# JuliaMLTools/GraphNets.jl

Measured on AMD Instinct MI355X. Metric: edges updated/sec, GNBlock fwd, 1M-edge batch, higher is better.
Workload: dtype f32; 1 GPU; C2: one shared Erdos-Renyi graph, 100k nodes / 1M edges, batch_size=1 (BASELINE configs[1]); dims=(10, 5, 0)=>(3, 4, 5), edges_whole_job=1000000, edges_per_gpu=1000000, nodes_per_gpu=100000, graphs_per_gpu=1, parallelism=single GPU

## Files before the change

### graphnets.jl_amd/csrc/gnx_device.h

```cpp
#pragma once
#ifndef GNX_JIT
#include <hip/hip_runtime.h>
#endif

namespace gnx {

struct Tile {
  int n0, n1;
  int e0, e1;
  int g;
  int win0;
  int win1;
  int flags;
};

constexpr int kPdRowsCap = 28;

struct BlockArgs {
  int de, dn, dg;
  int oe, on, og;
  const float *We, *be, *Wn, *bn, *Wg, *bg;
  int act_e, act_n, act_g;
  const float *ef, *nf, *gf;
  float *ef_out, *nf_out, *gf_out;
// ... 5 lines not shown
  const int* edge_off;
  const int* tile_off;
  const Tile* tiles;
  const int* wtile_off;
  const Tile* wtiles;
  int N, E, G, n_tiles, n_wtiles;
  const float* ln_g[3];
  const float* ln_b[3];
  float ln_eps;
  int ln_mode;
  const float* ln_stats[3];
  int ln_inline_e;
  const int* packs;
  int n_packs;
  const float *ffe_w1, *ffe_b1, *ffe_w2, *ffe_b2, *ffe_g2, *ffe_be2;
  int ffe_act1, ffe_act2;
  void* ffe_scratch;
  const float* prev_partials;
  const float* prev_gf;
  float* prev_gf_out;
  int prev_blocks;
};

struct RunSlot {
  const float *ef, *nf, *gf;
  float *ef_out, *nf_out, *gf_out;
  float* partials;
};
constexpr int kRunSlots = 8;
struct RunTable {
  RunSlot slot[kRunSlots];
};
constexpr unsigned kRunTableOffset = (unsigned)((sizeof(BlockArgs) + 7) / 8 * 8);

__device__ __forceinline__ float relu_f(float x) {
  float r;
  asm("v_max_f32 %0, 0, %1" : "=v"(r) : "v"(x));
  return r;
}

__device__ __forceinline__ float act_apply(float x, int act) {
  switch (act) {
    case 1: return relu_f(x);
    case 2: return tanhf(x);
    case 3: return 1.f / (1.f + expf(-x));
    case 4: return 0.5f * x * (1.f + tanhf(0.7978845608028654f * (x + 0.044715f * x * x * x)));
    default: return x;
  }
}

__device__ __forceinline__ float act_grad_from_out(float y, int act) {
  switch (act) {
    case 1: return y > 0.f ? 1.f : 0.f;
    case 2: return 1.f - y * y;
    case 3: return y * (1.f - y);
    default: return 1.f;
  }
}

__device__ __forceinline__ int segment_of(const int* cp, int n, int e) {
  int lo = 0, hi = n;
  while (hi - lo > 1) {
    const int mid = (lo + hi) >> 1;
    if (cp[mid] <= e) lo = mid; else hi = mid;
  }
  return lo;
// ... 10 lines not shown
```

### graphnets.jl_amd/csrc/gnx_forward.hip

```cpp
#include <algorithm>
#include <cstdlib>

#include "gnx_staging.h"
#include "gnx_step_hazard.h"

namespace gnx {

static_assert(GNX_ACT_IDENTITY == 0 && GNX_ACT_RELU == 1 && GNX_ACT_TANH == 2 && GNX_ACT_SIGMOID == 3 && GNX_ACT_GELU == 4,
              "act_apply (gnx_device.h) hard-codes the activation codes");

static int32_t check_block(const gnx_graphs* h, const gnx_block_params* p, int64_t R) {
  if (!h || !p) return fail(GNX_ERR_INVALID_ARG, "NULL handle or params");
  if (R <= 0) return fail(GNX_ERR_INVALID_ARG, "n_replicas must be >= 1");
  if (R > 1 && h->G != 1)
    return fail(GNX_ERR_INVALID_ARG, "n_replicas > 1 needs a single-graph handle (shared adjacency, batch.jl:66)");
  if (R > 65535) return fail(GNX_ERR_TOO_LARGE, "n_replicas exceeds the grid limit (65535)");
  const int d[6] = {p->de, p->dn, p->dg, p->oe, p->on, p->og};
  for (int i = 0; i < 6; ++i)
    if (d[i] < 0) return fail(GNX_ERR_DIMS, "negative feature width");
  if (p->de + p->dn + p->dg == 0) return fail(GNX_ERR_DIMS, "all input widths are 0 (gnblock.jl:48, batch.jl:56)");
  if (p->oe + p->on + p->og == 0) return fail(GNX_ERR_DIMS, "all output widths are 0 (gnblock.jl:49)");
  const gnx_dense* fn[3] = {&p->edgefn, &p->nodefn, &p->graphfn};
  const int out[3] = {p->oe, p->on, p->og};
  const int in[3] = {p->de + 2 * p->dn + p->dg, p->oe + p->dn + p->dg, p->oe + p->on + p->dg};
// ... 329 lines not shown
int32_t gnx_block_forward_chained(const gnx_graphs* h, const gnx_block_params* p, const float* ef, const float* nf, const float* gf, int64_t R, float* ef_out,
                                  float* nf_out, float* gf_out, void* ws, size_t ws_bytes, uint32_t flags, void* stream, const gnx_pending_update* prev,
                                  gnx_pending_update* pending) {
  if (!pending) return fail(GNX_ERR_INVALID_ARG, "pending is NULL");
  DeviceTurn turn((hipStream_t)stream, p && matrix_core_widths(*p));
  if (flags & GNX_FLAG_DEFER_GRAPH_UPDATE) return fail(GNX_ERR_INVALID_ARG, "gnx_block_forward_chained defers the graph update itself");
  return chained_step(BlockCall{h, p, GNX_ELEM_F32, ef, nf, gf, R, ef_out, nf_out, gf_out, ws, ws_bytes, flags, (hipStream_t)stream, GNX_PHASE_ALL}, prev, pending);
}

static StepSpans step_spans(const gnx_graphs* h, const gnx_block_params* p, int64_t R, const gnx_block_step& st, size_t elem, size_t ws_extent) {
  const void* const in[3] = {st.ef, st.nf, st.gf};
  const void* const out[3] = {st.ef_out, st.nf_out, st.gf_out};
  const long long rows[3] = {(long long)h->E, (long long)h->N, (long long)h->G};
  const int in_w[3] = {p->de, p->dn, p->dg}, out_w[3] = {p->oe, p->on, p->og};
  return step_spans_of(in, out, st.workspace, st.workspace_bytes, rows, in_w, out_w, R, elem, ws_extent);
}

static bool steps_overlap_applies(const gnx_graphs* h, const gnx_block_params* p, int64_t R, uint32_t flags, hipStream_t s) {
  if (!h || !p || matrix_core_widths(*p) || (flags & GNX_FLAG_FORCE_GENERIC) || form(GNX_FLAG_NO_FORK) || profile_enabled()) return false;
  if (check_block(h, p, R) != GNX_OK) return false;
  return block_narrow_takes(h, block_probe(h, p), s);
}

constexpr int kStepsRunDefault = 8;
static_assert(kRunMax == kRunSlots, "gnx_step_hazard.h groups what gnx_device.h's table holds");
static int steps_run_max() {
  static const int v = [] {
    const char* e = getenv("GNX_STEPS_RUN_MAX");
    const int n = e && *e ? atoi(e) : kStepsRunDefault;
    return n < 1 ? 1 : (n > kRunMax ? kRunMax : n);
  }();
  return v;
}

static int32_t steps_schedule(const gnx_graphs* h, const gnx_block_params* p, int32_t elem, const gnx_block_step* steps, int64_t n_steps, int64_t R,
                              uint32_t flags, void* stream, bool overlap) {
  const AuxHold hold = overlap ? take_aux(h, true) : AuxHold{};
  const gnx_graphs::AuxSet* aux = hold.set;
  const bool two = aux != nullptr;
  hipStream_t str[2] = {(hipStream_t)stream, aux ? aux->stream : nullptr};
  gnx_pending_update pend[2]{};
  auto flush = [&](int k) -> int32_t {
    if (!pend[k].workspace) return GNX_OK;
    const int32_t rc = graph_update(h, p, elem, pend[k], R, flags, str[k]);
    pend[k] = gnx_pending_update{};
    return rc;
  };
  auto run = [&](const gnx_block_step& st, int k, gnx_pending_update* next) -> int32_t {
    const gnx_pending_update* prev = pend[k].workspace ? &pend[k] : nullptr;
    return chained_step(BlockCall{h, p, elem, st.ef, st.nf, st.gf, R, st.ef_out, st.nf_out, st.gf_out, st.workspace, st.workspace_bytes, flags, str[k], GNX_PHASE_ALL},
                        prev, next);
  };
  const bool bf16 = elem == GNX_ELEM_BF16;
  const bool valid = h && p && check_block(h, p, R) == GNX_OK;
  const size_t elem_bytes = bf16 ? 2 : sizeof(float);
  const size_t ws_extent = !valid ? 0 : bf16 ? typed_ws(h, p, R, true).total : block_ws(h, p, R).total;
  bool can_fuse = valid && R == 1 && !(flags & GNX_FLAG_FORCE_GENERIC) && steps_run_max() > 1 && !profile_enabled();
  auto slot_of = [&](const gnx_block_step& st, RunSlot& sl, BlockArgs* run_args) -> bool {
    Prepared q(BlockCall{h, p, elem, st.ef, st.nf, st.gf, R, st.ef_out, st.nf_out, st.gf_out, st.workspace, st.workspace_bytes, flags, str[0], GNX_PHASE_ALL});
    if (q.rc) return false;
    if (run_args) {
      if (!block_narrow_run_applies(h, q.a, bf16)) return can_fuse = false;
      *run_args = q.a;
    }
    sl = RunSlot{q.a.ef, q.a.nf, q.a.gf, q.a.ef_out, q.a.nf_out, q.a.gf_out, q.a.partials};
    return true;
  };
  if (two) {
    GNX_HIP(hipEventRecord(aux->fork, str[0]));
    GNX_HIP(hipStreamWaitEvent(str[1], aux->fork, 0));
  }
  RunSpans recent[3];
  int32_t rc = GNX_OK;
  int64_t i = 0;
  for (int64_t j = 0; i < n_steps && rc == GNX_OK; ++j) {
    const gnx_block_step& st = steps[i];
    RunSpans cur;
    RunTable tab{};
    BlockArgs run_args{};
    cur.step[0] = valid ? step_spans(h, p, R, st, elem_bytes, ws_extent) : StepSpans{};
    cur.n = 1;
    if (can_fuse && n_steps - i >= 2) {
      RunSpans win = cur;
      while (i + win.n < n_steps) {
        const StepSpans sp = step_spans(h, p, R, steps[i + win.n], elem_bytes, ws_extent);
        if (!run_takes(win, sp, steps_run_max())) break;
        win.step[win.n++] = sp;
      }
      bool ok = window_is_run(win.n, i, n_steps, steps_run_max());
      for (int z = 0; ok && z < win.n; ++z) ok = slot_of(steps[i + z], tab.slot[z], z == 0 ? &run_args : nullptr);
      if (ok) cur = win;
    }
    const int k = two ? (int)(j & 1) : 0, o = k ^ 1;
    StepOrder ord;
    if (two) {
      ord = run_order(cur, recent, j);
    } else {
      ord.flush_own = pend[0].workspace && (pend[0].workspace == st.workspace || (p && p->og > 0 && pend[0].gf_out == st.gf_out) || runs_conflict(cur, recent[0]));
    }
    if ((ord.flush_own || cur.n > 1) && (rc = flush(k))) break;
    if (two && j >= 3) {
      const hipError_t e = hipStreamWaitEvent(str[k], aux->step[(j - 3) & 3], 0);
      if (e != hipSuccess) { rc = hip_fail(e, "gnx_block_forward_steps: ordering a step behind the step three before it"); break; }
    }
    if (ord.after_other) {
      if ((rc = flush(o))) break;
      hipEvent_t ev = o == 1 ? aux->join : aux->fork;
      hipError_t e = hipEventRecord(ev, str[o]);
      if (e == hipSuccess) e = hipStreamWaitEvent(str[k], ev, 0);
      if (e != hipSuccess) { rc = hip_fail(e, "gnx_block_forward_steps: ordering a step behind the other stream"); break; }
    }
    if (cur.n > 1) {
      rc = launch_block_narrow_run(h, run_args, tab, cur.n, str[k], bf16);
    } else {
      gnx_pending_update next{};
      rc = run(st, k, &next);
      if (rc == GNX_OK) pend[k] = next;
    }
    if (rc != GNX_OK) break;
    if (two) {
      if (const hipError_t e = hipEventRecord(aux->step[j & 3], str[k]); e != hipSuccess) { rc = hip_fail(e, "gnx_block_forward_steps: step event"); break; }
    }
    recent[2] = recent[1]; recent[1] = recent[0]; recent[0] = cur;
    i += cur.n;
  }
  const int32_t rf0 = flush(0), rf1 = two ? flush(1) : GNX_OK;
  hipError_t e1 = hipSuccess, e2 = hipSuccess;
  if (two) {
    e1 = hipEventRecord(aux->join, str[1]);
    e2 = hipStreamWaitEvent(str[0], aux->join, 0);
  }
  if (rc) return rc;
  if (rf0) return rf0;
  if (rf1) return rf1;
  GNX_HIP(e1);
  GNX_HIP(e2);
  return GNX_OK;
}

int32_t gnx_block_forward_steps(const gnx_graphs* h, const gnx_block_params* p, const gnx_block_step* steps, int64_t n_steps, int64_t R, uint32_t flags,
                                void* stream) {
  if (n_steps < 0 || (n_steps > 0 && !steps)) return fail(GNX_ERR_INVALID_ARG, "gnx_block_forward_steps: steps is NULL / n_steps is negative");
  if (flags & GNX_FLAG_DEFER_GRAPH_UPDATE) return fail(GNX_ERR_INVALID_ARG, "gnx_block_forward_steps finishes every step's graph update itself");
  DeviceTurn turn((hipStream_t)stream, p && matrix_core_widths(*p));
  FormScope forms(flags);
  return steps_schedule(h, p, GNX_ELEM_F32, steps, n_steps, R, flags, stream, n_steps > 1 && steps_overlap_applies(h, p, R, flags, (hipStream_t)stream));
}

int32_t gnx_block_forward_steps_typed(const gnx_graphs* h, const gnx_block_params* p, int32_t elem, const gnx_block_step* steps, int64_t n_steps, int64_t R,
                                      uint32_t flags, void* stream) {
  if (elem == GNX_ELEM_F32) return gnx_block_forward_steps(h, p, steps, n_steps, R, flags, stream);
  if (elem != GNX_ELEM_BF16) return fail(GNX_ERR_INVALID_ARG, "elem must be GNX_ELEM_F32 or GNX_ELEM_BF16");
  if (flags & GNX_FLAG_DEFER_GRAPH_UPDATE) return fail(GNX_ERR_INVALID_ARG, "gnx_block_forward_steps_typed finishes every step's graph update itself");
  if (n_steps < 0 || (n_steps > 0 && !steps)) return fail(GNX_ERR_INVALID_ARG, "gnx_block_forward_steps_typed: steps is NULL / n_steps is negative");
  for (int64_t i = 0; i < n_steps; ++i) {
    const gnx_block_step& st = steps[i];
    const void* bufs[6] = {st.ef, st.nf, st.gf, st.ef_out, st.nf_out, st.gf_out};
    for (const void* b : bufs)
      if (((uintptr_t)b & 3) != 0) return fail(GNX_ERR_INVALID_ARG, "bf16 feature buffers must be 4-byte aligned (in every step)");
  }
  const hipStream_t s = (hipStream_t)stream;
  DeviceTurn turn(s, p && matrix_core_widths(*p));
  FormScope forms(flags);
  if (!h || !p || check_block(h, p, R) != GNX_OK || !typed_native(h, p, flags, s)) {
    for (int64_t i = 0; i < n_steps; ++i) {
// ... 428 lines not shown
```

### graphnets.jl_amd/csrc/gnx_launchers.h

```cpp
#pragma once
#include "gnx_internal.h"

namespace gnx {

struct EdgeLaunch {
  const Tile* tiles; size_t n_tiles; const float* ef; size_t E;
  struct { const float* stats; const float* g; const float* b; bool inline_stats; float eps; int mode; } ln;
  const float* We; int ldw;
  const float* psrc;
  const float* pdst;
  size_t N; const int* src; const int* dst; int act;
  float* out; float* colsum;
  float* agg_out; size_t n_agg_rows; const int* chunk_row0;
  int64_t R; void* scratch; hipStream_t stream;
};

int32_t launch_block_generic(const BlockArgs& a, int64_t R, int tile_n_cap, hipStream_t s, int phase);
int32_t launch_layernorm2(const float* x, size_t rows, int d, const gnx_layernorm& l1, const gnx_layernorm& l2, float eps, int eps_mode, float* y1, float* y2, hipStream_t s);
int32_t launch_layernorm2_bf16(const void* x, size_t rows, int d, const gnx_layernorm& l1, const gnx_layernorm& l2, float eps, int eps_mode, float* y1, float* y2, hipStream_t s);
int32_t launch_ffn_residual(const float* z, const float* x, size_t rows, int d, const gnx_ffn& ff, float* out, hipStream_t s);
int32_t launch_pad(const gnx_graphs* h, int kind, bool pad, const float* src, int d, int64_t R, float* dst, hipStream_t s);
int32_t launch_calibration(int n, hipStream_t s);
int xent_blocks(int64_t cols);
int32_t launch_xent_backward(const float* logits, const float* targets, int d, int64_t cols, const float* upstream, float* dl, hipStream_t s);
int32_t launch_xent(const float* logits, const float* targets, int d, int64_t cols, float* out, float* ws, hipStream_t s);
int32_t launch_collapse(const gnx_graphs* h, const float* ef, int d, int64_t R, float* out, hipStream_t s);
int32_t launch_collapse_padded(const gnx_graphs* h, const float* ef, int d, int64_t R, float* out, hipStream_t s);
int32_t launch_fn_input(const gnx_graphs* h, int kind, const float* ef, int de, const float* nf, int dn, const float* gf, int dg, int64_t R, float* out, hipStream_t s,
                        bool bf16 = false);

int32_t launch_block_narrow(const gnx_graphs* h, const BlockArgs& a, int64_t R, hipStream_t s, int phase, bool bf16 = false);
void warm_block_narrow(const gnx_graphs* h, const gnx_block_params* p, bool bf16 = false);
bool block_narrow_ready(const gnx_graphs* h, const BlockArgs& a, hipStream_t s);
bool block_narrow_ffe_applies(const gnx_graphs* h, const BlockArgs& a, int act1, int act2);
bool block_narrow_chain_applies(const gnx_graphs* h, const BlockArgs& a, bool bf16 = false);
bool block_narrow_takes(const gnx_graphs* h, const BlockArgs& a, hipStream_t s, bool bf16 = false);
int32_t launch_block_narrow_chained(const gnx_graphs* h, const BlockArgs& a, int64_t R, hipStream_t s, bool bf16);
bool narrow_bf16_aot(const gnx_graphs* h, const BlockArgs& a);
int32_t launch_fused_bf16(const gnx_graphs* h, const BlockArgs& a, int64_t R, hipStream_t s, int phase);
int32_t launch_chained_bf16(const gnx_graphs* h, const BlockArgs& a, int64_t R, hipStream_t s);
bool narrow_bf16_ln_aot(const gnx_graphs* h, const BlockArgs& a);
int32_t launch_ln_bf16(const gnx_graphs* h, const BlockArgs& a, int64_t R, hipStream_t s, int phase);
bool block_narrow_run_applies(const gnx_graphs* h, const BlockArgs& a, bool bf16);
bool narrow_bf16_run(const gnx_graphs* h, const BlockArgs& a);
int32_t launch_block_narrow_run(const gnx_graphs* h, const BlockArgs& a, const RunTable& t, int Z, hipStream_t s, bool bf16);
int32_t launch_run_bf16(const gnx_graphs* h, const BlockArgs& a, const RunTable& t, int Z, hipStream_t s);
bool jit_eligible(const BlockArgs& a, int ept);
int32_t jit_get(const BlockArgs& a, int ept, hipStream_t s, hipFunction_t* block, hipFunction_t* graph, bool bf16 = false);
int32_t jit_get_core_post3(int d0, int d1, int d2, hipStream_t s, hipFunction_t* fn);

bool core_narrow_width(int d);
int32_t launch_ln1_rows(const float* x, size_t rows, int d, const gnx_layernorm& l1, float eps, int eps_mode, float* y, hipStream_t s);
bool core_post3_applies(const size_t rows[3], const int d[3], const gnx_ffn ff[3], bool deferred, hipStream_t s);
int32_t launch_core_post3(const float* const x[3], const size_t rows[3], const int d[3], const gnx_layernorm l2[3], const gnx_ffn ff[3], float eps,
                          int eps_mode, float* const out[3], hipStream_t s, const BlockArgs* blk, int n_rows, bool skip_edges = false,
                          const float* const block_out[3] = nullptr);
int32_t launch_core_post(const float* x, size_t rows, int d, const gnx_layernorm& l2, const gnx_ffn& ff, float eps, int eps_mode, float* out, hipStream_t s,
                         const float* block_out = nullptr);

int32_t launch_block_wide(const gnx_graphs* h, const BlockArgs& a, int64_t R, hipStream_t s, int phase);
size_t wide_workspace_bytes(const gnx_graphs* h, const gnx_block_params* p, int64_t R);
void warm_block_wide(const gnx_graphs* h, const gnx_block_params* p, bool rows_gemm);
bool block_wide_ln_applies(const gnx_graphs* h, const BlockArgs& a);
bool block_wide_edge_x6_applies(const gnx_graphs* h, const BlockArgs& a);
int32_t launch_dense_rows(const gnx_graphs* h, int entity, const float* A, int K, const gnx_dense& d, int OUT, const float* add1,
                          const float* add2, float* out, int64_t R, hipStream_t s, const char* name);
int32_t launch_rows_matmul(const gnx_graphs* h, int entity, const float* A, int K, const float* B, int ldw, int OUT, float* out, int64_t R,
                           hipStream_t s, const char* name, const float* gmul, int gmul_act, float* tile_colsum, int* n_tiles_out, const float* add1);

int32_t launch_ffn_fused(const gnx_graphs* h, int entity, const float* z, int d, const gnx_ffn& ff, const float* add1, const float* add2, float* out,
                         int64_t R, hipStream_t s, const float* ln_stats = nullptr, const gnx_layernorm* ln = nullptr, void* scratch = nullptr, size_t scratch_bytes = 0,
                         bool ln_inline = false, float ln_eps = 0.f, int ln_mode = 0);
bool ffn_fused_applies(const float* z, int d, const gnx_ffn& ff, const float* add1, const float* add2, const float* out);
bool ln_stats_applies(const float* x, int d);
int32_t launch_ln_stats(const float* x, size_t rows, int d, float eps, int eps_mode, float* stats, hipStream_t s);
bool ffn_x6_applies(const float* z, int d, const gnx_ffn& ff, const float* add1, const float* add2, const float* out, size_t scratch_bytes);
int32_t launch_ffn_x6(const float* z, size_t nrows, int d, const gnx_ffn& ff, const float* add1, const float* add2, float* out, int64_t R, hipStream_t s,
                      const float* ln_stats, const gnx_layernorm* ln, void* scratch, bool ln_inline, float ln_eps, int ln_mode);
// ... 80 lines not shown
```

### graphnets.jl_amd/csrc/gnx_narrow.hip

```cpp
#include <cstdlib>

#include "gnx_launchers.h"
#include "gnx_narrow_launch.h"
#include "gnx_wave_kernel.h"

namespace gnx {

#define GNX_NARROW_DIMS(X) \
  X(10, 5, 0, 3, 4)        \
  X(3, 4, 5, 3, 4)         \
  X(10, 5, 3, 3, 4)        \
  X(0, 2, 0, 2, 2)         \
  X(2, 2, 2, 2, 2)         \
  X(4, 3, 2, 3, 4)         \
  X(8, 8, 8, 16, 8)        \
  X(10, 5, 3, 10, 5)       \
  X(10, 5, 0, 10, 5)
static bool narrow_aot_listed(const BlockArgs& a) {
#define GNX_CASE(DE, DN, DG, OE, ON) \
  if (a.de == DE && a.dn == DN && a.dg == DG && a.oe == OE && a.on == ON) return true;
  GNX_NARROW_DIMS(GNX_CASE)
#undef GNX_CASE
  return false;
}
// ... 68 lines not shown
  a.prev_blocks = a.prev_partials ? (h->G == 1 ? 1 : (int)((h->G + 3) / 4)) : 0;
  if (bf16) {
    const int32_t rc = launch_chained_bf16(h, a, R, s);
    return rc == 1 ? fail(GNX_ERR_INVALID_ARG, "internal: chained bf16 launch for a width set without that kernel") : rc;
  }
#define GNX_CASE(DE, DN, DG, OE, ON)                                                                                               \
  if (a.de == DE && a.dn == DN && a.dg == DG && a.oe == OE && a.on == ON) {                                                         \
    if constexpr (OE + ON > 0) {                                                                                                   \
      return h->G == 1 ? launch_wave_g<DE, DN, DG, OE, ON, 2, false, true, false, true>(h, a, R, s, 1)                              \
                       : launch_wave_g<DE, DN, DG, OE, ON, 2, false, false, false, true>(h, a, R, s, 1);                            \
    }                                                                                                                              \
  }
  GNX_NARROW_DIMS(GNX_CASE)
#undef GNX_CASE
  return fail(GNX_ERR_INVALID_ARG, "internal: chained launch for a width set without that kernel");
}

#define GNX_NARROW_RUN_DIMS(X) \
  X(10, 5, 0, 3, 4)            \
  X(3, 4, 5, 3, 4)             \
  X(10, 5, 3, 3, 4)            \
  X(0, 2, 0, 2, 2)             \
  X(2, 2, 2, 2, 2)             \
  X(4, 3, 2, 3, 4)
bool block_narrow_run_applies(const gnx_graphs* h, const BlockArgs& a, bool bf16) {
  if (!block_narrow_chain_applies(h, a, bf16)) return false;
  if (bf16) return narrow_bf16_run(h, a);
#define GNX_CASE(DE, DN, DG, OE, ON) \
  if (a.de == DE && a.dn == DN && a.dg == DG && a.oe == OE && a.on == ON) return true;
  GNX_NARROW_RUN_DIMS(GNX_CASE)
#undef GNX_CASE
  return false;
}
int32_t launch_block_narrow_run(const gnx_graphs* h, const BlockArgs& a, const RunTable& t, int Z, hipStream_t s, bool bf16) {
  if (bf16) {
    const int32_t rc = launch_run_bf16(h, a, t, Z, s);
    return rc == 1 ? fail(GNX_ERR_INVALID_ARG, "internal: bf16 run launch for a width set without that kernel") : rc;
  }
#define GNX_CASE(DE, DN, DG, OE, ON)                                                                                               \
  if (a.de == DE && a.dn == DN && a.dg == DG && a.oe == OE && a.on == ON) {                                                         \
    if constexpr (OE + ON > 0) {                                                                                                   \
      return h->G == 1 ? launch_wave_run<DE, DN, DG, OE, ON, true>(h, a, t, Z, s) : launch_wave_run<DE, DN, DG, OE, ON, false>(h, a, t, Z, s); \
    }                                                                                                                              \
  }
  GNX_NARROW_RUN_DIMS(GNX_CASE)
#undef GNX_CASE
  return fail(GNX_ERR_INVALID_ARG, "internal: run launch for a width set without that kernel");
}

bool block_narrow_ffe_applies(const gnx_graphs* h, const BlockArgs& a, int act1, int act2) {
  return ln_aot(h, a) && a.ln_g[0] && act1 <= GNX_ACT_RELU && act2 <= GNX_ACT_RELU && a.act_e <= GNX_ACT_RELU && h->max_in_degree <= h->wtile_e_cap &&
         !form(GNX_FLAG_NO_FFE);
}

enum NarrowRoute { NR_NONE, NR_AOT, NR_JIT };
static NarrowRoute narrow_route(const gnx_graphs* h, const BlockArgs& a, hipStream_t s, bool bf16 = false) {
  if (a.n_wtiles == 0 || a.E == 0 || wants_ln(a)) return NR_NONE;
  auto jit_ok = [&]() {
    const int ept = jit_ept(h);
    hipFunction_t fb, fg;
    return ept && jit_get(a, ept, s, &fb, &fg, bf16) == GNX_OK;
  };
  static const bool jit_all = getenv("GNX_JIT_ALL") != nullptr;
  if (jit_all && jit_ok()) return NR_JIT;
  if (bf16) {
    if (narrow_bf16_aot(h, a)) return NR_AOT;
  } else if (narrow_aot_listed(a)) {
    return h->wtile_e_cap == 64 || h->wtile_e_cap == 128 || (h->wtile_e_cap == 256 && (a.de + a.dn) * 4 <= 64) ? NR_AOT : NR_NONE;
  }
  return jit_ok() ? NR_JIT : NR_NONE;
}

bool block_narrow_takes(const gnx_graphs* h, const BlockArgs& a, hipStream_t s, bool bf16) { return narrow_route(h, a, s, bf16) != NR_NONE; }

int32_t launch_block_narrow(const gnx_graphs* h, const BlockArgs& a, int64_t R, hipStream_t s, int phase, bool bf16) {
  if (a.n_wtiles == 0 || a.E == 0) return 1;
  if (wants_ln(a)) {
    if (bf16) {
      const int32_t rc = launch_ln_bf16(h, a, R, s, phase);
      return rc == 1 ? fail(GNX_ERR_INVALID_ARG, "internal: LayerNorm-on-load on bf16 rows for a width set without that kernel") : rc;
// ... 25 lines not shown
```

### graphnets.jl_amd/csrc/gnx_narrow_launch.h

```cpp
#pragma once
#include <cstdlib>

#include "gnx_device.h"
#include "gnx_wave_kernel.h"

namespace gnx {

static int partial_rows(const gnx_graphs* h) { return (int)(h->G == 1 ? (h->n_wtiles() + 3) / 4 : h->n_wtiles()); }

static int graph_update_threads(const gnx_graphs* h) {
  return graph_update_threads_for_rows(h->G == 1 ? (h->n_wtiles() + 3) / 4 : h->max_wtiles_per_graph);
}

template <int DE, int DN, int DG, int OE, int ON, int EPT, bool LN, bool ONEG, bool FFE = false, bool CHAIN = false, bool BF16 = false>
static int32_t launch_wave_g(const gnx_graphs* h, const BlockArgs& a, int64_t R, hipStream_t s, int phase) {
  constexpr int C = OE + ON;
  const int n_rows = partial_rows(h);
  const unsigned grid = (unsigned)((a.n_wtiles + 3) / 4) + (CHAIN ? (unsigned)a.prev_blocks : 0u);
  if (phase & 1) {
    ProfScope ps("k_block_wave", s);
#ifdef GNX_WAVE_STAMPS_BUILD
    static unsigned long long* d_dbg = nullptr;
    static size_t dbg_cap = 0;
    const char* dump = getenv("GNX_WAVE_STAMPS_DUMP");
    if (dump) {
      if (dbg_cap < (size_t)a.n_wtiles) { if (d_dbg) (void)hipFree(d_dbg); dbg_cap = (size_t)a.n_wtiles; (void)hipMalloc((void**)&d_dbg, dbg_cap * 64); }
      (void)hipMemsetAsync(d_dbg, 0, (size_t)a.n_wtiles * 64, s);
      (void)hipMemcpyToSymbolAsync(HIP_SYMBOL(g_wave_dbg), &d_dbg, sizeof(d_dbg), 0, hipMemcpyHostToDevice, s);
    }
#endif
    if constexpr (FFE) GNX_LAUNCH((k_block_wave_ffe<DE, DN, DG, OE, ON, EPT, ONEG, BF16>), dim3(grid, (unsigned)R), dim3(kThreads), 0, s, a, n_rows);
    else GNX_LAUNCH((k_block_wave<DE, DN, DG, OE, ON, EPT, LN, ONEG, false, false, CHAIN, BF16>), dim3(grid, (unsigned)R), dim3(kThreads), 0, s, a, n_rows);
    GNX_HIP(hipGetLastError());
#ifdef GNX_WAVE_STAMPS_BUILD
    if (dump) {
      (void)hipStreamSynchronize(s);
      std::vector<unsigned long long> hs((size_t)a.n_wtiles * 8);
      (void)hipMemcpy(hs.data(), d_dbg, hs.size() * 8, hipMemcpyDeviceToHost);
      if (FILE* f = fopen(dump, "wb")) { fwrite(hs.data(), 8, hs.size(), f); fclose(f); }
    }
#endif
  }
  if ((phase & 2) && a.og > 0) {
    if constexpr (C > 0) {
      const int threads = graph_update_threads(h);
      const size_t lds = sizeof(float) * (size_t)graph_update_lds_floats(C, a.dg, a.og, threads);
      ProfScope ps("k_graph_t", s);
      GNX_LAUNCH((k_graph_t<C, ONEG, BF16, BF16 && !LN>), dim3((unsigned)a.G, (unsigned)R), dim3(threads), lds, s, a, n_rows);
      GNX_HIP(hipGetLastError());
    }
  }
  return GNX_OK;
}

template <int DE, int DN, int DG, int OE, int ON, bool ONEG, bool BF16 = false>
static int32_t launch_wave_run(const gnx_graphs* h, const BlockArgs& a, const RunTable& t, int Z, hipStream_t s) {
  constexpr int C = OE + ON;
  if (Z < 1 || Z > kRunSlots) return fail(GNX_ERR_INVALID_ARG, "internal: a run of more steps than the table has slots");
  const int n_rows = partial_rows(h);
  {
    ProfScope ps("k_block_wave", s);
    GNX_LAUNCH((k_block_wave_run<DE, DN, DG, OE, ON, 2, ONEG, BF16>), dim3((unsigned)((a.n_wtiles + 3) / 4), (unsigned)Z), dim3(kThreads), 0, s, a, t, n_rows);
    GNX_HIP(hipGetLastError());
  }
  if (a.og > 0) {
    const int threads = graph_update_threads(h);
    const size_t lds = sizeof(float) * (size_t)graph_update_lds_floats(C, a.dg, a.og, threads);
    ProfScope ps("k_graph_t", s);
    GNX_LAUNCH((k_graph_run<C, ONEG, BF16>), dim3((unsigned)a.G, (unsigned)Z), dim3(threads), lds, s, a, t, n_rows);
    GNX_HIP(hipGetLastError());
  }
  return GNX_OK;
}

template <int DE, int DN, int DG, int OE, int ON, int EPT, bool BF16 = false>
static bool launch_wave_pack(const gnx_graphs* h, const BlockArgs& a, int64_t R, hipStream_t s, int phase, int32_t* rc) {
  constexpr int C = OE + ON;
  if constexpr (EPT != 2 || C == 0) return false;
  else {
    if (h->G <= 1 || h->n_packs <= 0 || !a.packs || phase != 3 || a.og <= 0 || form(GNX_FLAG_NO_PACK)) return false;
    ProfScope ps("k_block_wave", s);
    GNX_LAUNCH((k_block_wave<DE, DN, DG, OE, ON, EPT, false, false, true, false, false, BF16>), dim3((unsigned)h->n_packs, (unsigned)R), dim3(kPackThreads), 0, s, a, 0);
    const hipError_t e = hipGetLastError();
    *rc = e == hipSuccess ? GNX_OK : hip_fail(e, "k_block_wave<PACK>");
    return true;
  }
}

template <int DE, int DN, int DG, int OE, int ON, int EPT, bool LN = false, bool BF16 = false>
static int32_t launch_wave_t(const gnx_graphs* h, const BlockArgs& a, int64_t R, hipStream_t s, int phase) {
  if constexpr (!LN) {
    int32_t rc = GNX_OK;
    if (launch_wave_pack<DE, DN, DG, OE, ON, EPT, BF16>(h, a, R, s, phase, &rc)) return rc;
  }
  return h->G == 1 ? launch_wave_g<DE, DN, DG, OE, ON, EPT, LN, true, false, false, BF16>(h, a, R, s, phase)
                   : launch_wave_g<DE, DN, DG, OE, ON, EPT, LN, false, false, false, BF16>(h, a, R, s, phase);
}

template <int DE, int DN, int DG, int OE, int ON, bool BF16 = false>
static int32_t launch_fused(const gnx_graphs* h, const BlockArgs& a, int64_t R, hipStream_t s, int phase) {
  if (h->wtile_e_cap == 64) return launch_wave_t<DE, DN, DG, OE, ON, 1, false, BF16>(h, a, R, s, phase);
  if (h->wtile_e_cap == 128) return launch_wave_t<DE, DN, DG, OE, ON, 2, false, BF16>(h, a, R, s, phase);
  if (h->wtile_e_cap == 256) {
    if constexpr ((DE + DN) * 4 <= 64) return launch_wave_t<DE, DN, DG, OE, ON, 4, false, BF16>(h, a, R, s, phase);
// ... 6 lines not shown
```

### graphnets.jl_amd/csrc/gnx_step_hazard.h

```cpp
#pragma once
#include <cstddef>
#include <cstdint>

namespace gnx {

struct ByteSpan {
  uintptr_t lo = 0, hi = 0;
};

inline ByteSpan byte_span(const void* p, size_t bytes) {
  ByteSpan s;
  if (p && bytes) { s.lo = reinterpret_cast<uintptr_t>(p); s.hi = s.lo + bytes; }
  return s;
}

inline bool spans_overlap(ByteSpan a, ByteSpan b) { return a.lo < a.hi && b.lo < b.hi && a.lo < b.hi && b.lo < a.hi; }

struct StepSpans {
  ByteSpan rd[3];
  ByteSpan wr[4];
};

inline StepSpans step_spans_of(const void* const in[3], const void* const out[3], const void* ws, size_t ws_bytes, const long long rows[3],
                               const int in_w[3], const int out_w[3], long long R, size_t elem, size_t ws_extent) {
// ... 42 lines not shown
  return false;
}

inline bool runs_conflict(const RunSpans& x, const RunSpans& y) {
  for (int b = 0; b < y.n; ++b)
    if (run_conflicts_step(x, y.step[b])) return true;
  return false;
}

inline bool run_takes(const RunSpans& run, const StepSpans& next, int run_max) {
  return run.n >= 1 && run.n < run_max && run.n < kRunMax && !run_conflicts_step(run, next);
}

inline bool window_is_run(int n, long long first, long long n_steps, int run_max) {
  return n >= 2 && (n == run_max || (first + n == n_steps && n >= kRunTailMin));
}

inline RunSpans group_run(const StepSpans* spans, long long n_steps, long long first, int run_max) {
  RunSpans run;
  if (first >= n_steps) return run;
  run.step[run.n++] = spans[first];
  while (first + run.n < n_steps && run_takes(run, spans[first + run.n], run_max)) { run.step[run.n] = spans[first + run.n]; ++run.n; }
  if (!window_is_run(run.n, first, n_steps, run_max)) run.n = 1;
  return run;
}

inline StepOrder run_order(const RunSpans& cur, const RunSpans* recent, long long j) {
  StepOrder o;
  o.flush_own = j >= 2 && runs_conflict(cur, recent[1]);
  o.after_other = (j >= 1 && runs_conflict(cur, recent[0])) || (j >= 3 && runs_conflict(cur, recent[2]));
  return o;
}

}
```

### graphnets.jl_amd/csrc/gnx_wave_kernel.h

```cpp
#pragma once
#include "gnx_device.h"

namespace gnx {

namespace {

constexpr int kThreads = 256;

struct __attribute__((packed, aligned(4))) F4u { float x, y, z, w; };
struct __attribute__((packed, aligned(4))) F3u { float x, y, z; };
struct __attribute__((packed, aligned(4))) F2u { float x, y; };

typedef const float __attribute__((address_space(4))) * cfloatp;
__device__ __forceinline__ cfloatp as_const(const float* p) { return reinterpret_cast<cfloatp>(reinterpret_cast<size_t>(p)); }

template <int D>
__device__ __forceinline__ void load_row(const float* __restrict__ p, float (&x)[D > 0 ? D : 1]) {
  constexpr int Q = D / 4, R = D % 4;
#pragma unroll
  for (int q = 0; q < Q; ++q) {
    const F4u v = *reinterpret_cast<const F4u*>(p + 4 * q);
    x[4 * q] = v.x; x[4 * q + 1] = v.y; x[4 * q + 2] = v.z; x[4 * q + 3] = v.w;
  }
  if constexpr (R == 3) {
// ... 609 lines not shown
#ifndef GNX_WAVE_PK
#define GNX_WAVE_PK 1
#endif
#ifndef GNX_WAVE_SGPRS
#define GNX_WAVE_SGPRS 80
#endif
#ifdef GNX_WAVE_STAMPS_BUILD
static __device__ unsigned long long* g_wave_dbg = nullptr;
#define GNX_WSTAMP(i) do { __builtin_amdgcn_sched_barrier(0); wst_[i] = clock64(); __builtin_amdgcn_sched_barrier(0); } while (0)
#else
#define GNX_WSTAMP(i) do { } while (0)
#endif
constexpr int kPackThreads = 512;
typedef const BlockArgs __attribute__((address_space(4))) * cargsp;
template <bool FRESH>
__device__ __forceinline__ auto phase_args(const BlockArgs& a) {
  if constexpr (FRESH) {
    cargsp p = (cargsp)__builtin_amdgcn_kernarg_segment_ptr();
    asm volatile("" : "+s"(p));
    return p;
  } else {
    return &a;
  }
}

typedef const RunSlot __attribute__((address_space(4))) * cslotp;
__device__ __forceinline__ cslotp run_slot() {
  typedef const char __attribute__((address_space(4))) * ccharp;
  cslotp p = (cslotp)((ccharp)__builtin_amdgcn_kernarg_segment_ptr() + kRunTableOffset) + blockIdx.y;
  asm volatile("" : "+s"(p));
  return p;
}

template <int DE, int DN, int DG, int OE, int ON, int EPT, bool LN, bool ONEG, bool PACK, bool FFE, bool CHAIN, bool BF16 = false, bool RUN = false, bool OUT32 = false>
__device__ __forceinline__ void block_wave_body(BlockArgs& a, int n_rows) {
  static_assert(!OUT32 || (BF16 && LN), "OUT32: bf16 rows in, fp32 rows out — the LayerNorm-on-load block of a bf16 core");
  constexpr bool OBF16 = BF16 && !OUT32;
  static_assert(!RUN || (!PACK && !FFE && !LN && !CHAIN && OE + ON > 0), "RUN: the two-launch form of a plain block, one slot per step");
  static_assert(!(PACK && ONEG), "packs are for batches of several graphs");
  static_assert(!BF16 || OUT32 || (!FFE && !LN), "bf16 features: the plain block forward and its chained form; a core's block hands on fp32");
  static_assert(!CHAIN || (!PACK && !FFE && !LN && OE + ON > 0), "CHAIN: the two-launch form of a plain block");
  static_assert(!FFE || (LN && DE == OE && DE > 0 && EPT == 2 && (DE + DN) * OE > 96 && ((DE + DN) * OE) % 2 == 0 && GNX_WAVE_PK && !PACK),
                "FFE: a core's block (dims => dims) with LayerNorm on load, two edges per lane, streamed weights");
  constexpr int OE1 = OE > 0 ? OE : 1, ON1 = ON > 0 ? ON : 1, DE1 = DE > 0 ? DE : 1, DN1 = DN > 0 ? DN : 1, DG1 = DG > 0 ? DG : 1;
  constexpr int TEW = 64 * EPT;
  constexpr int C = OE + ON, C1 = C > 0 ? C : 1;
  constexpr int WAVES = (PACK ? kPackThreads : kThreads) / 64;
  constexpr int WSL = wave_slice_floats(OE, EPT);
  constexpr bool FRESH = FFE || (CHAIN && BF16 && !ONEG);
  __shared__ __attribute__((aligned(16))) float s_mem[WAVES * WSL];

  const int lane = threadIdx.x & 63;
  const int wv = __builtin_amdgcn_readfirstlane(threadIdx.x >> 6);
  typedef const int __attribute__((address_space(4))) * cintp;
  int bx = blockIdx.x, gx = gridDim.x;
  if constexpr (CHAIN) {
    if ((int)blockIdx.x < a.prev_blocks) {
      if (a.og > 0) {
        constexpr int CPc = (C + 3) / 4 * 4;
        const float* pbase = a.prev_partials + blockIdx.y * (size_t)n_rows * CPc;
        if constexpr (ONEG) {
          const int rows = (a.n_wtiles + 3) / 4;
          graph_update_rows<C, false, 4, BF16>(a, a.prev_gf, a.prev_gf_out, pbase, 0, blockIdx.y, 0, rows, (int)threadIdx.x, kThreads, s_mem, graph_update_threads_for_rows(rows));
        } else {
          const int g = (int)blockIdx.x * WAVES + wv;
          if (g < a.G) graph_update_rows<C, true, 4, BF16>(a, a.prev_gf, a.prev_gf_out, pbase, g, blockIdx.y, a.wtile_off[g], a.wtile_off[g + 1], lane, 64, s_mem + wv * WSL);
        }
      }
      return;
    }
    bx -= a.prev_blocks; gx -= a.prev_blocks;
  }
  int wt;
  if constexpr (PACK) {
    const cintp pk = reinterpret_cast<cintp>(reinterpret_cast<size_t>(a.packs)) + (size_t)xcd_tile(bx, gx) * WAVES;
    wt = pk[wv];
  } else {
    wt = __builtin_amdgcn_readfirstlane(xcd_tile(bx, gx) * WAVES + wv);
  }
  const bool active = PACK ? wt >= 0 : wt < a.n_wtiles;
  int tile_g = -1, tile_cnt = 0;
  bool owner = false;
#ifdef GNX_WAVE_STAMPS_BUILD
  unsigned long long wst_[8] = {0, 0, 0, 0, 0, 0, 0, 0};
#endif
  GNX_WSTAMP(0);
  if constexpr (!ONEG && !PACK) { if (!active) return; }
  float mine = 0.f;
  float xr[FFE ? EPT : 1][FFE ? DE1 : 1];
// ... 380 lines not shown
#pragma unroll
      for (int m = 0; m < EPT; ++m) {
        float o[DE1];
#pragma unroll
        for (int k = 0; k < DE; ++k) o[k] = m == 0 ? acc2[k].x : acc2[k].y;
        if (ffe_act2 == 1) {
#pragma unroll
          for (int k = 0; k < DE; ++k) o[k] = relu_f(o[k]);
        }
#pragma unroll
        for (int k = 0; k < DE; ++k) o[k] = rs[m][k] + o[k];
        if (ffv[m]) store_row<OE>(feat<BF16>(ef_out_t) + (ff_row0 + 64 * m) * OE, o);
      }
    }
  }
}

template <int DE, int DN, int DG, int OE, int ON, int EPT, bool LN = false, bool ONEG = false, bool PACK = false, bool FFE = false, bool CHAIN = false,
          bool BF16 = false>
__global__ __launch_bounds__(PACK ? kPackThreads : kThreads) __attribute__((amdgpu_num_sgpr(GNX_WAVE_SGPRS))) void k_block_wave(BlockArgs a, int n_rows) {
  static_assert(!FFE, "the FFE form is k_block_wave_ffe");
  block_wave_body<DE, DN, DG, OE, ON, EPT, LN, ONEG, PACK, false, CHAIN, BF16, false, LN && BF16>(a, n_rows);
}
template <int DE, int DN, int DG, int OE, int ON, int EPT, bool ONEG, bool BF16 = false>
__global__ __launch_bounds__(kThreads) __attribute__((amdgpu_waves_per_eu(4))) void k_block_wave_ffe(BlockArgs a, int n_rows) {
  block_wave_body<DE, DN, DG, OE, ON, EPT, true, ONEG, false, true, false, BF16, false, BF16>(a, n_rows);
}

template <int DE, int DN, int DG, int OE, int ON, int EPT, bool ONEG, bool BF16 = false>
__global__ __launch_bounds__(kThreads) __attribute__((amdgpu_num_sgpr(GNX_WAVE_SGPRS))) void k_block_wave_run(BlockArgs a, RunTable t, int n_rows) {
  block_wave_body<DE, DN, DG, OE, ON, EPT, false, ONEG, false, false, false, BF16, true>(a, n_rows);
}

template <int C, bool ONEG = false, bool BF16 = false, bool OBF16 = BF16>
__global__ void k_graph_t(BlockArgs a, int n_rows) {
  extern __shared__ float s_g[];
  constexpr int CP = (C + 3) / 4 * 4;
  const int g = blockIdx.x;
  const int t0 = ONEG ? 0 : a.wtile_off[g], t1 = ONEG ? (a.n_wtiles + 3) / 4 : a.wtile_off[g + 1];
  const float* base = a.partials + blockIdx.y * (size_t)n_rows * CP;
  if (blockDim.x == 64) graph_update_rows<C, true, 16, BF16, OBF16>(a, a.gf, a.gf_out, base, g, blockIdx.y, t0, t1, (int)threadIdx.x, 64, s_g);
  else graph_update_rows<C, false, 16, BF16, OBF16>(a, a.gf, a.gf_out, base, g, blockIdx.y, t0, t1, (int)threadIdx.x, (int)blockDim.x, s_g);
}

template <int C, bool ONEG = false, bool BF16 = false>
__global__ void k_graph_run(BlockArgs a, RunTable t, int n_rows) {
  extern __shared__ float s_g[];
  const int g = blockIdx.x;
  const int t0 = ONEG ? 0 : a.wtile_off[g], t1 = ONEG ? (a.n_wtiles + 3) / 4 : a.wtile_off[g + 1];
  const cslotp S = run_slot();
  const float* const base = S->partials;
  const float* const gf = S->gf;
  float* const gf_out = S->gf_out;
  if (blockDim.x == 64) graph_update_rows<C, true, 16, BF16>(a, gf, gf_out, base, g, 0, t0, t1, (int)threadIdx.x, 64, s_g);
  else graph_update_rows<C, false, 16, BF16>(a, gf, gf_out, base, g, 0, t0, t1, (int)threadIdx.x, (int)blockDim.x, s_g);
}

}
```

Before: 58.20 billion edges/s.

## Defer a fused run's graph update into the next run's block kernel

When consecutive multi-step runs are issued on the two-stream schedule, the graph-update phase of one run is held back. It is then executed by extra leading blocks of the next run's edge/node kernel, through a new PrevTable passed in kernargs after the RunTable. Partials alternate between two workspace areas so the deferred update can still read the previous run's partials while the next run writes its own. This removes one kernel launch and one inter-run serialization point per run, at the cost of more hazard-checking logic, a new kernel variant, and the risk of ordering or aliasing mistakes between the deferred and the current step.

```diff
diff --git a/graphnets.jl_amd/csrc/gnx_device.h b/graphnets.jl_amd/csrc/gnx_device.h
--- a/graphnets.jl_amd/csrc/gnx_device.h
+++ b/graphnets.jl_amd/csrc/gnx_device.h
@@ -61,6 +61,18 @@
   RunSlot slot[kRunSlots];
 };
 constexpr unsigned kRunTableOffset = (unsigned)((sizeof(BlockArgs) + 7) / 8 * 8);
+struct PrevSlot {
+  const float* gf;
+  float* gf_out;
+  const float* partials;
+};
+struct PrevTable {
+  PrevSlot slot[kRunSlots];
+  int n;
+  int per_slot;
+};
+constexpr unsigned kPrevTableOffset = kRunTableOffset + (unsigned)sizeof(RunTable);
+static_assert(sizeof(RunTable) % 8 == 0, "the PrevTable follows the RunTable without padding");
 
 __device__ __forceinline__ float relu_f(float x) {
   float r;
diff --git a/graphnets.jl_amd/csrc/gnx_forward.hip b/graphnets.jl_amd/csrc/gnx_forward.hip
--- a/graphnets.jl_amd/csrc/gnx_forward.hip
+++ b/graphnets.jl_amd/csrc/gnx_forward.hip
@@ -385,6 +385,15 @@
   }();
   return v;
 }
+
+static bool steps_defer_on() {
+  static const bool v = [] {
+    const char* e = getenv("GNX_STEPS_DEFER");
+    return !(e && *e && atoi(e) == 0);
+  }();
+  return v;
+}
+static int partial_rows_of(const gnx_graphs* h);
 
 static int32_t steps_schedule(const gnx_graphs* h, const gnx_block_params* p, int32_t elem, const gnx_block_step* steps, int64_t n_steps, int64_t R,
                               uint32_t flags, void* stream, bool overlap) {
@@ -424,6 +433,24 @@
     GNX_HIP(hipStreamWaitEvent(str[1], aux->fork, 0));
   }
   RunSpans recent[3];
+  int rstream[3] = {0, 0, 0};
+  struct RunPending {
+    bool has = false;
+    BlockArgs args;
+    RunTable tab;
+    int n = 0, area = 0, stream = 0;
+    int64_t j = 0;
+  } rpend;
+  const BlockWs bw = valid && !bf16 ? block_ws(h, p, R) : BlockWs{};
+  const bool area_b_fits = valid && !bf16 && bw.part_off - bw.agg_off >= sizeof(float) * (size_t)partial_rows_of(h) * (size_t)((p->oe + p->on + 3) / 4 * 4);
+  const bool can_defer = two && !bf16 && area_b_fits && steps_defer_on();
+  auto flush_run = [&]() -> int32_t {
+    if (!rpend.has) return GNX_OK;
+    rpend.has = false;
+    if (const int32_t frc = launch_block_narrow_run(h, rpend.args, rpend.tab, rpend.n, str[rpend.stream], false, GNX_PHASE_GRAPH)) return frc;
+    if (const hipError_t e = hipEventRecord(aux->step[rpend.j & 3], str[rpend.stream]); e != hipSuccess) return hip_fail(e, "gnx_block_forward_steps: step event");
+    return GNX_OK;
+  };
   int32_t rc = GNX_OK;
   int64_t i = 0;
   for (int64_t j = 0; i < n_steps && rc == GNX_OK; ++j) {
@@ -444,10 +471,15 @@
       for (int z = 0; ok && z < win.n; ++z) ok = slot_of(steps[i + z], tab.slot[z], z == 0 ? &run_args : nullptr);
       if (ok) cur = win;
     }
-    const int k = two ? (int)(j & 1) : 0, o = k ^ 1;
+    const bool carry_kernel = can_defer && cur.n > 1 && block_narrow_carry_applies(h, run_args);
+    const bool carries = rpend.has && carry_kernel && run_defers(cur, recent[0]);
+    if (!carries && (rc = flush_run())) break;
+    const RunPlace place = two ? run_place(j, carries, rstream) : RunPlace{};
+    const int k = place.stream, o = k ^ 1;
     StepOrder ord;
     if (two) {
-      ord = run_order(cur, recent, j);
+      if (place.regular) ord = run_order(cur, recent, j);
+      else ord.flush_own = ord.after_other = true;
     } else {
       ord.flush_own = pend[0].workspace && (pend[0].workspace == st.workspace || (p && p->og > 0 && pend[0].gf_out == st.gf_out) || runs_conflict(cur, recent[0]));
     }
@@ -464,7 +496,22 @@
       if (e != hipSuccess) { rc = hip_fail(e, "gnx_block_forward_steps: ordering a step behind the other stream"); break; }
     }
     if (cur.n > 1) {
-      rc = launch_block_narrow_run(h, run_args, tab, cur.n, str[k], bf16);
+      if (carries) {
+        PrevTable prev{};
+        prev.n = rpend.n;
+        for (int z = 0; z < rpend.n; ++z) prev.slot[z] = PrevSlot{rpend.tab.slot[z].gf, rpend.tab.slot[z].gf_out, rpend.tab.slot[z].partials};
+        const int area = rpend.area ^ 1;
+        if (area == 1)
+          for (int z = 0; z < cur.n; ++z) tab.slot[z].partials = reinterpret_cast<float*>(static_cast<char*>(steps[i + z].workspace) + bw.agg_off);
+        rpend.has = false;
+        rc = launch_block_narrow_carry(h, run_args, tab, cur.n, prev, str[k]);
+        if (rc == GNX_OK) { rpend.has = true; rpend.args = run_args; rpend.tab = tab; rpend.n = cur.n; rpend.area = area; rpend.stream = k; rpend.j = j; }
+      } else if (carry_kernel) {
+        rc = launch_block_narrow_run(h, run_args, tab, cur.n, str[k], false, GNX_PHASE_EDGE_NODE);
+        if (rc == GNX_OK) { rpend.has = true; rpend.args = run_args; rpend.tab = tab; rpend.n = cur.n; rpend.area = 0; rpend.stream = k; rpend.j = j; }
+      } else {
+        rc = launch_block_narrow_run(h, run_args, tab, cur.n, str[k], bf16);
+      }
     } else {
       gnx_pending_update next{};
       rc = run(st, k, &next);
@@ -475,8 +522,10 @@
       if (const hipError_t e = hipEventRecord(aux->step[j & 3], str[k]); e != hipSuccess) { rc = hip_fail(e, "gnx_block_forward_steps: step event"); break; }
     }
     recent[2] = recent[1]; recent[1] = recent[0]; recent[0] = cur;
+    rstream[2] = rstream[1]; rstream[1] = rstream[0]; rstream[0] = k;
     i += cur.n;
   }
+  const int32_t rfr = flush_run();
   const int32_t rf0 = flush(0), rf1 = two ? flush(1) : GNX_OK;
   hipError_t e1 = hipSuccess, e2 = hipSuccess;
   if (two) {
@@ -484,6 +533,7 @@
     e2 = hipStreamWaitEvent(str[0], aux->join, 0);
   }
   if (rc) return rc;
+  if (rfr) return rfr;
   if (rf0) return rf0;
   if (rf1) return rf1;
   GNX_HIP(e1);
diff --git a/graphnets.jl_amd/csrc/gnx_launchers.h b/graphnets.jl_amd/csrc/gnx_launchers.h
--- a/graphnets.jl_amd/csrc/gnx_launchers.h
+++ b/graphnets.jl_amd/csrc/gnx_launchers.h
@@ -43,7 +43,9 @@
 int32_t launch_ln_bf16(const gnx_graphs* h, const BlockArgs& a, int64_t R, hipStream_t s, int phase);
 bool block_narrow_run_applies(const gnx_graphs* h, const BlockArgs& a, bool bf16);
 bool narrow_bf16_run(const gnx_graphs* h, const BlockArgs& a);
-int32_t launch_block_narrow_run(const gnx_graphs* h, const BlockArgs& a, const RunTable& t, int Z, hipStream_t s, bool bf16);
+int32_t launch_block_narrow_run(const gnx_graphs* h, const BlockArgs& a, const RunTable& t, int Z, hipStream_t s, bool bf16, int phase = 3);
+bool block_narrow_carry_applies(const gnx_graphs* h, const BlockArgs& a);
+int32_t launch_block_narrow_carry(const gnx_graphs* h, const BlockArgs& a, const RunTable& t, int Z, const PrevTable& prev, hipStream_t s);
 int32_t launch_run_bf16(const gnx_graphs* h, const BlockArgs& a, const RunTable& t, int Z, hipStream_t s);
 bool jit_eligible(const BlockArgs& a, int ept);
 int32_t jit_get(const BlockArgs& a, int ept, hipStream_t s, hipFunction_t* block, hipFunction_t* graph, bool bf16 = false);
diff --git a/graphnets.jl_amd/csrc/gnx_narrow.hip b/graphnets.jl_amd/csrc/gnx_narrow.hip
--- a/graphnets.jl_amd/csrc/gnx_narrow.hip
+++ b/graphnets.jl_amd/csrc/gnx_narrow.hip
@@ -124,20 +124,49 @@
 #undef GNX_CASE
   return false;
 }
-int32_t launch_block_narrow_run(const gnx_graphs* h, const BlockArgs& a, const RunTable& t, int Z, hipStream_t s, bool bf16) {
-  if (bf16) {
+int32_t launch_block_narrow_run(const gnx_graphs* h, const BlockArgs& a, const RunTable& t, int Z, hipStream_t s, bool bf16, int phase) {
+  if (bf16) {
+    if (phase != 3) return fail(GNX_ERR_INVALID_ARG, "internal: a bf16 run is issued whole");
     const int32_t rc = launch_run_bf16(h, a, t, Z, s);
     return rc == 1 ? fail(GNX_ERR_INVALID_ARG, "internal: bf16 run launch for a width set without that kernel") : rc;
   }
 #define GNX_CASE(DE, DN, DG, OE, ON)                                                                                               \
   if (a.de == DE && a.dn == DN && a.dg == DG && a.oe == OE && a.on == ON) {                                                         \
     if constexpr (OE + ON > 0) {                                                                                                   \
-      return h->G == 1 ? launch_wave_run<DE, DN, DG, OE, ON, true>(h, a, t, Z, s) : launch_wave_run<DE, DN, DG, OE, ON, false>(h, a, t, Z, s); \
+      return h->G == 1 ? launch_wave_run<DE, DN, DG, OE, ON, true>(h, a, t, Z, s, phase) : launch_wave_run<DE, DN, DG, OE, ON, false>(h, a, t, Z, s, phase); \
     }                                                                                                                              \
   }
   GNX_NARROW_RUN_DIMS(GNX_CASE)
 #undef GNX_CASE
   return fail(GNX_ERR_INVALID_ARG, "internal: run launch for a width set without that kernel");
+}
+
+#define GNX_NARROW_CARRY_DIMS(X1, XG) \
+  X1(10, 5, 0, 3, 4) XG(10, 5, 0, 3, 4) \
+  X1(3, 4, 5, 3, 4) XG(3, 4, 5, 3, 4)   \
+  X1(10, 5, 3, 3, 4) XG(10, 5, 3, 3, 4) \
+  X1(0, 2, 0, 2, 2) XG(0, 2, 0, 2, 2)   \
+  X1(4, 3, 2, 3, 4) XG(4, 3, 2, 3, 4)
+bool block_narrow_carry_applies(const gnx_graphs* h, const BlockArgs& a) {
+  if (!block_narrow_run_applies(h, a, false)) return false;
+#define GNX_CASE1(DE, DN, DG, OE, ON) \
+  if (h->G == 1 && a.de == DE && a.dn == DN && a.dg == DG && a.oe == OE && a.on == ON) return true;
+#define GNX_CASEG(DE, DN, DG, OE, ON) \
+  if (h->G != 1 && a.de == DE && a.dn == DN && a.dg == DG && a.oe == OE && a.on == ON) return true;
+  GNX_NARROW_CARRY_DIMS(GNX_CASE1, GNX_CASEG)
+#undef GNX_CASE1
+#undef GNX_CASEG
+  return false;
+}
+int32_t launch_block_narrow_carry(const gnx_graphs* h, const BlockArgs& a, const RunTable& t, int Z, const PrevTable& prev, hipStream_t s) {
+#define GNX_CASE1(DE, DN, DG, OE, ON) \
+  if (h->G == 1 && a.de == DE && a.dn == DN && a.dg == DG && a.oe == OE && a.on == ON) return launch_wave_carry<DE, DN, DG, OE, ON, true>(h, a, t, Z, prev, s);
+#define GNX_CASEG(DE, DN, DG, OE, ON) \
+  if (h->G != 1 && a.de == DE && a.dn == DN && a.dg == DG && a.oe == OE && a.on == ON) return launch_wave_carry<DE, DN, DG, OE, ON, false>(h, a, t, Z, prev, s);
+  GNX_NARROW_CARRY_DIMS(GNX_CASE1, GNX_CASEG)
+#undef GNX_CASE1
+#undef GNX_CASEG
+  return fail(GNX_ERR_INVALID_ARG, "internal: carrying run launch for a width set without that kernel");
 }
 
 bool block_narrow_ffe_applies(const gnx_graphs* h, const BlockArgs& a, int act1, int act2) {
diff --git a/graphnets.jl_amd/csrc/gnx_narrow_launch.h b/graphnets.jl_amd/csrc/gnx_narrow_launch.h
--- a/graphnets.jl_amd/csrc/gnx_narrow_launch.h
+++ b/graphnets.jl_amd/csrc/gnx_narrow_launch.h
@@ -54,22 +54,37 @@
 }
 
 template <int DE, int DN, int DG, int OE, int ON, bool ONEG, bool BF16 = false>
-static int32_t launch_wave_run(const gnx_graphs* h, const BlockArgs& a, const RunTable& t, int Z, hipStream_t s) {
+static int32_t launch_wave_run(const gnx_graphs* h, const BlockArgs& a, const RunTable& t, int Z, hipStream_t s, int phase = 3) {
   constexpr int C = OE + ON;
   if (Z < 1 || Z > kRunSlots) return fail(GNX_ERR_INVALID_ARG, "internal: a run of more steps than the table has slots");
   const int n_rows = partial_rows(h);
-  {
+  if (phase & 1) {
     ProfScope ps("k_block_wave", s);
     GNX_LAUNCH((k_block_wave_run<DE, DN, DG, OE, ON, 2, ONEG, BF16>), dim3((unsigned)((a.n_wtiles + 3) / 4), (unsigned)Z), dim3(kThreads), 0, s, a, t, n_rows);
     GNX_HIP(hipGetLastError());
   }
-  if (a.og > 0) {
+  if ((phase & 2) && a.og > 0) {
     const int threads = graph_update_threads(h);
     const size_t lds = sizeof(float) * (size_t)graph_update_lds_floats(C, a.dg, a.og, threads);
     ProfScope ps("k_graph_t", s);
     GNX_LAUNCH((k_graph_run<C, ONEG, BF16>), dim3((unsigned)a.G, (unsigned)Z), dim3(threads), lds, s, a, t, n_rows);
     GNX_HIP(hipGetLastError());
   }
+  return GNX_OK;
+}
+
+template <int DE, int DN, int DG, int OE, int ON, bool ONEG>
+static int32_t launch_wave_carry(const gnx_graphs* h, const BlockArgs& a0, const RunTable& t, int Z, const PrevTable& prev0, hipStream_t s) {
+  if (Z < 1 || Z > kRunSlots || prev0.n < 1 || prev0.n > kRunSlots) return fail(GNX_ERR_INVALID_ARG, "internal: a run of more steps than the table has slots");
+  BlockArgs a = a0;
+  PrevTable prev = prev0;
+  prev.per_slot = h->G == 1 ? 1 : (int)((h->G + 3) / 4);
+  a.prev_blocks = ((h->G == 1 ? prev.n : prev.per_slot * ((prev.n + Z - 1) / Z)) + 7) / 8 * 8;
+  const int n_rows = partial_rows(h);
+  ProfScope ps("k_block_wave", s);
+  GNX_LAUNCH((k_block_wave_carry<DE, DN, DG, OE, ON, 2, ONEG>), dim3((unsigned)((a.n_wtiles + 3) / 4) + (unsigned)a.prev_blocks, (unsigned)Z), dim3(kThreads), 0, s, a, t,
+             prev, n_rows);
+  GNX_HIP(hipGetLastError());
   return GNX_OK;
 }
 
diff --git a/graphnets.jl_amd/csrc/gnx_step_hazard.h b/graphnets.jl_amd/csrc/gnx_step_hazard.h
--- a/graphnets.jl_amd/csrc/gnx_step_hazard.h
+++ b/graphnets.jl_amd/csrc/gnx_step_hazard.h
@@ -98,4 +98,40 @@
   return o;
 }
 
+inline bool spans_identical(ByteSpan a, ByteSpan b) { return a.lo == b.lo && a.hi == b.hi; }
+
+inline bool step_defers(const StepSpans& x, const StepSpans& y) {
+  for (int t = 0; t < 4; ++t) {
+    for (const ByteSpan& r : y.rd) if (spans_overlap(x.wr[t], r)) return false;
+    for (int u = 0; u < 4; ++u) {
+      if (!spans_overlap(x.wr[t], y.wr[u])) continue;
+      const bool rows = t < 2 && u < 2, gf_out = t == 2 && u == 2, ws = t == 3 && u == 3 && spans_identical(x.wr[3], y.wr[3]);
+      if (!rows && !gf_out && !ws) return false;
+    }
+  }
+  for (const ByteSpan& w : y.wr)
+    for (const ByteSpan& r : x.rd) if (spans_overlap(w, r)) return false;
+  return true;
 }
+
+inline bool run_defers(const RunSpans& cur, const RunSpans& prev) {
+  if (cur.n < 2 || prev.n < 2 || !runs_conflict(cur, prev)) return false;
+  for (int a = 0; a < cur.n; ++a)
+    for (int b = 0; b < prev.n; ++b)
+      if (!step_defers(cur.step[a], prev.step[b])) return false;
+  return true;
+}
+
+struct RunPlace {
+  int stream = 0;
+  bool regular = true;
+};
+inline RunPlace run_place(long long j, bool carries, const int* recent_stream) {
+  RunPlace p;
+  p.stream = carries ? recent_stream[0] : (int)(j & 1);
+  p.regular = p.stream == (int)(j & 1);
+  for (int d = 1; d <= 3 && d <= j; ++d) p.regular = p.regular && recent_stream[d - 1] == (int)((j - d) & 1);
+  return p;
+}
+
+}
diff --git a/graphnets.jl_amd/csrc/gnx_wave_kernel.h b/graphnets.jl_amd/csrc/gnx_wave_kernel.h
--- a/graphnets.jl_amd/csrc/gnx_wave_kernel.h
+++ b/graphnets.jl_amd/csrc/gnx_wave_kernel.h
@@ -665,11 +665,20 @@
   return p;
 }
 
+typedef const PrevTable __attribute__((address_space(4))) * cprevp;
+__device__ __forceinline__ cprevp run_prev() {
+  typedef const char __attribute__((address_space(4))) * ccharp;
+  cprevp p = (cprevp)((ccharp)__builtin_amdgcn_kernarg_segment_ptr() + kPrevTableOffset);
+  asm volatile("" : "+s"(p));
+  return p;
+}
+
 template <int DE, int DN, int DG, int OE, int ON, int EPT, bool LN, bool ONEG, bool PACK, bool FFE, bool CHAIN, bool BF16 = false, bool RUN = false, bool OUT32 = false>
 __device__ __forceinline__ void block_wave_body(BlockArgs& a, int n_rows) {
   static_assert(!OUT32 || (BF16 && LN), "OUT32: bf16 rows in, fp32 rows out — the LayerNorm-on-load block of a bf16 core");
   constexpr bool OBF16 = BF16 && !OUT32;
-  static_assert(!RUN || (!PACK && !FFE && !LN && !CHAIN && OE + ON > 0), "RUN: the two-launch form of a plain block, one slot per step");
+  static_assert(!RUN || (!PACK && !FFE && !LN && OE + ON > 0), "RUN: the two-launch form of a plain block, one slot per step");
+  static_assert(!(RUN && CHAIN) || !BF16, "RUN with a CHAIN front (k_block_wave_carry): fp32 rows only");
   static_assert(!(PACK && ONEG), "packs are for batches of several graphs");
   static_assert(!BF16 || OUT32 || (!FFE && !LN), "bf16 features: the plain block forward and its chained form; a core's block hands on fp32");
   static_assert(!CHAIN || (!PACK && !FFE && !LN && OE + ON > 0), "CHAIN: the two-launch form of a plain block");
@@ -687,7 +696,33 @@
   const int wv = __builtin_amdgcn_readfirstlane(threadIdx.x >> 6);
   typedef const int __attribute__((address_space(4))) * cintp;
   int bx = blockIdx.x, gx = gridDim.x;
-  if constexpr (CHAIN) {
+  if constexpr (CHAIN && RUN) {
+    if constexpr (ONEG) {
+      gx = (a.n_wtiles + 3) / 4;
+      if (bx >= gx) {
+        if (a.og > 0 && blockIdx.y == 0) {
+          const cprevp P = run_prev();
+          if (const int z = bx - gx; z < P->n) {
+            graph_update_rows<C, false, 4, BF16>(a, P->slot[z].gf, P->slot[z].gf_out, P->slot[z].partials, 0, 0, 0, gx, (int)threadIdx.x, kThreads, s_mem,
+                                                 graph_update_threads_for_rows(gx));
+          }
+        }
+        return;
+      }
+    } else {
+      if (bx < a.prev_blocks) {
+        if (a.og > 0) {
+          const cprevp P = run_prev();
+          const int q = bx / P->per_slot;
+          const int g = (bx - q * P->per_slot) * WAVES + wv;
+          if (const int z = (int)blockIdx.y + q * (int)gridDim.y; z < P->n && g < a.G)
+            graph_update_rows<C, true, 4, BF16>(a, P->slot[z].gf, P->slot[z].gf_out, P->slot[z].partials, g, 0, a.wtile_off[g], a.wtile_off[g + 1], lane, 64, s_mem + wv * WSL);
+        }
+        return;
+      }
+      bx -= a.prev_blocks; gx -= a.prev_blocks;
+    }
+  } else if constexpr (CHAIN) {
     if ((int)blockIdx.x < a.prev_blocks) {
       if (a.og > 0) {
         constexpr int CPc = (C + 3) / 4 * 4;
@@ -1134,6 +1169,11 @@
   block_wave_body<DE, DN, DG, OE, ON, EPT, false, ONEG, false, false, false, BF16, true>(a, n_rows);
 }
 
+template <int DE, int DN, int DG, int OE, int ON, int EPT, bool ONEG>
+__global__ __launch_bounds__(kThreads) __attribute__((amdgpu_num_sgpr(GNX_WAVE_SGPRS))) void k_block_wave_carry(BlockArgs a, RunTable t, PrevTable pt, int n_rows) {
+  block_wave_body<DE, DN, DG, OE, ON, EPT, false, ONEG, false, false, true, false, true>(a, n_rows);
+}
+
 template <int C, bool ONEG = false, bool BF16 = false, bool OBF16 = BF16>
 __global__ void k_graph_t(BlockArgs a, int n_rows) {
   extern __shared__ float s_g[];
```

Result: faster. 60.09 billion edges/s, median of 6 (+3.2%).
